# RamSaw/PipelineDP

Hardware: AMD Instinct MI355X
Metric: records/sec DPEngine.aggregate COUNT+SUM at 1/2/4/8 MI355X; % HBM roofline (higher is better)
Workload: dtype f64; 1 GPU; configs[1]: 1e+09 records / 1e+07 privacy ids / 1e+06 Zipf(1.1) partitions per GPU, COUNT+SUM+PRIVACY_ID_COUNT, private partition selection; records_per_gpu=1000000000, privacy_ids_per_gpu=10000000, partitions=1000000, max_partitions_contributed=8, max_contributions_per_partition=2, noise=laplace, selection=truncated_geometric, parallelism=pid-sharded x1, privacy_id_range_supplied=True

## Files before the change

pipelinedp_amd/csrc/dpg_api.hip:

```cpp
#include <dlfcn.h>
#include <hip/hip_runtime.h>
#include <rccl/rccl.h>

#include <algorithm>
#include <cstddef>
#include <chrono>
#include <cmath>
#include <cstdio>
#include <cstdlib>
#include <cstring>
#include <map>
#include <mutex>
#include <string>
#include <thread>
#include <tuple>
#include <vector>

static hipError_t occ_query(int *blocks, const void *kern, int threads, size_t lds) {
    static std::mutex mu;
    static std::map<std::tuple<int, const void *, int, size_t>, int> cache;
    int dev = 0;
    (void)hipGetDevice(&dev);
    std::lock_guard<std::mutex> g(mu);
    const auto key = std::make_tuple(dev, kern, threads, lds);
    const auto it = cache.find(key);
    if (it != cache.end()) {
        *blocks = it->second;
        return hipSuccess;
    }
    const hipError_t e = hipOccupancyMaxActiveBlocksPerMultiprocessor(blocks, kern, threads, lds);
    if (e == hipSuccess) cache[key] = *blocks;
    return e;
}
static hipError_t set_func_attr(const void *kern, hipFuncAttribute attr, int value) {
    if (attr != hipFuncAttributeMaxDynamicSharedMemorySize) return hipFuncSetAttribute(kern, attr, value);
    static std::mutex mu;
    static std::map<std::pair<int, const void *>, int> done;
    int dev = 0;
    (void)hipGetDevice(&dev);
    std::lock_guard<std::mutex> g(mu);
    const auto key = std::make_pair(dev, kern);
    const auto it = done.find(key);
    if (it != done.end() && it->second >= value) return hipSuccess;
    const hipError_t e = hipFuncSetAttribute(kern, attr, value);
    if (e == hipSuccess) done[key] = value;
    return e;
}

#include "dpg_bound.h"
#include "dpg_chunk.h"
#include "dpg_common.h"
#include "dpg_hist.h"
#include "dpg_keydict.h"
#include "dpg_strkey.h"
#include "dpg_owner.h"
#include "dpg_pairx.h"
#include "dpg_partition.h"
#include "dpg_quantile.h"
#include "dpg_records.h"
#include "dpg_rsort.h"
#include "dpg_sample.h"
#include "dpg_select.h"
#include "dpg_shard.h"
#include "dpg_sortb.h"
#include "dpg_sortmw.h"
#include "dpg_team.h"
#include "dpg_utility.h"
#include "dpg_vsum.h"
#include "dpg_wave.h"
#include "dpg_hist_phases.h"

using namespace dpg;

namespace {

constexpr uint32_t kBucketTarget = 256;
constexpr uint32_t kMaxB1 = 11, kMaxB2 = 12, kMaxBR = 11;
constexpr uint32_t kMaxB1W = 12;
constexpr int kIptL1W = 8;
constexpr uint32_t kPinErr = 4096;
constexpr uint32_t kChunkGroup = 32;
constexpr int kRedoLevel2 = -100;
#ifndef DPG_PC_HALF
#define DPG_PC_HALF 0
#endif
#ifndef DPG_IPT_PC
#define DPG_IPT_PC 8
#endif

struct Buf {
    void *p = nullptr;
    size_t bytes = 0;
};

struct Control {
    uint32_t err;
    uint32_t item_cursor;
    uint32_t ntiles[8];
    int64_t n_scalar;
    uint32_t n_chunks;
    uint32_t n_over;
    uint32_t n_over2;
    uint32_t n_mchunks;
    uint32_t heavy_nfb;
    uint32_t pad_;
    uint32_t seg_paths[2];
    unsigned long long over_records;
    unsigned long long over2_records;
    unsigned long long pid_lo, pid_hi;
};

}

struct dpg_ctx {
    int device = 0;
    uint64_t seed = 0;
    int n_cu = 256;
    std::string err;
    std::map<std::string, Buf> bufs;
    std::vector<std::string> stage_names;
    std::vector<hipEvent_t> events;
    int n_events_used = 0;
    hipStream_t last_stream = nullptr;
    uint32_t bucket_target = 0;
    uint32_t bucket_cap = kBCap;
    void *comm = nullptr;
    const uint32_t *last_err = nullptr;
    int rank = 0, nranks = 1;
    char *stage_buf = nullptr;
    size_t stage_cap = 0, stage_head = 0;
    std::map<hipStream_t, hipEvent_t> stage_done;
    uint32_t *pin_tot = nullptr;
    hipEvent_t tot_ev = nullptr;
    uint32_t team_backoff = 0;
    uint32_t team_backoff_next = 64;
};

namespace {

int watchdog_seconds() {
#if defined(DPG_WATCHDOG) || defined(DPG_PHASE_TIMING)
    const char *e = std::getenv("DPG_WATCHDOG_S");
    return e ? std::atoi(e) : 0;
#else
    return 0;
#endif
}

uint32_t *watchdog_buffer(size_t n) {
    static uint32_t *buf = nullptr;
    static size_t cap = 0;
    if (n > cap) {
        if (buf) (void)hipHostFree(buf);
        if (hipHostMalloc((void **)&buf, n * 4, hipHostMallocCoherent) != hipSuccess) return nullptr;
        cap = n;
    }
    std::memset(buf, 0, n * 4);
    return buf;
}

void watchdog_wait(hipStream_t s, const uint32_t *prog, size_t n, const char *what) {
    int secs = watchdog_seconds();
    for (int i = 0; i < secs * 100; ++i) {
        if (hipStreamQuery(s) == hipSuccess) return;
        std::this_thread::sleep_for(std::chrono::milliseconds(10));
    }
    std::fprintf(stderr, "[dpg watchdog] %s did not finish in %d s; phases:", what, secs);
    for (size_t i = 0; i < n; ++i) std::fprintf(stderr, " %u", prog[i]);
    std::fprintf(stderr, "\n");
    std::fflush(stderr);
    std::abort();
// ... 972 lines not shown
    const uint32_t i = blockIdx.x * blockDim.x + threadIdx.x;
    if (i >= 8 * F) return;
    const uint32_t x = i / F, d = i % F;
    rbase[i] = ((int64_t)d * 8 + x) * C;
}

__global__ __launch_bounds__(1024) void k_piece_totals(const uint32_t *cum, const int64_t *rbase,
                                                       uint32_t F, uint32_t *tot, uint32_t *ptot,
                                                       int64_t *ostart, PieceDesc *desc) {
    __shared__ uint32_t sh[16];
    constexpr int DPT = 4;
    const uint32_t d0 = DPT * threadIdx.x;
    uint32_t c[DPT], x = 0;
#pragma unroll
    for (int u = 0; u < DPT; ++u) {
        c[u] = 0;
        uint32_t cp = 0;
        if (d0 + u < F) {
            const uint32_t d = d0 + u;
            const int64_t b0 = rbase[d];
            PieceDesc &pd = desc[d];
            for (int r = 0; r < 8; ++r) {
                const uint32_t y = cum[(size_t)r * F + d];
                pd.ppre[r] = cp;
                pd.dl[r] = (uint32_t)(rbase[(size_t)r * F + d] - b0) - cp;
                pd.cend[r] = cp + y;
                c[u] += y;
                cp += (y + 1u) & ~1u;
            }
            pd.n = cp;
            pd.base0 = b0;
            ptot[d] = cp;
        }
        x += c[u];
    }
    uint32_t total;
    uint32_t e = block_excl_scan_1024(x, sh, total);
#pragma unroll
    for (int u = 0; u < DPT; ++u) {
        if (d0 + u < F) {
            tot[d0 + u] = c[u];
            ostart[d0 + u] = e;
            desc[d0 + u].ostart = e;
        }
        e += c[u];
    }
}

uint32_t piece_capacity(int64_t n, uint32_t F, int64_t sub) {
    double c = 1.25 * (double)n / (8.0 * F) + 4096.0;
    if (const char *e = std::getenv("DPG_DEBUG_PIECE_CAP")) c = std::max(2.0, std::atof(e));
    const double slots = c * 8.0 * F + (double)sub;
    if (slots >= 4294967295.0) return 0;
    return (uint32_t)c & ~1u;
}

template <class R, int IPT, int FMAX, int NT = kScatThreads>
int run_level1_pieces(dpg_ctx *ctx, hipStream_t s, const SrcSoAKey<R, true> &src, int64_t n,
                      uint32_t F, uint32_t bits, uint32_t C, R *out, Control *ctl,
                      PieceTab *pt, uint32_t *host_tot) {
    int st = DPG_OK;
    if (n < 2) return fail(ctx, DPG_ERR_HIP, "internal: piece level needs two records");
    const int64_t sub = (int64_t)NT * IPT;
    const uint32_t nt = (uint32_t)((n + sub - 1) / sub);
    WS(tiles, TileDesc, "pieces.tiles", nt);
    WS(stb, uint32_t, "pieces.stb", 1);
    WS(snt, uint32_t, "pieces.snt", 1);
    WS(rbase, int64_t, "pieces.rbase", (size_t)8 * F);
    WS(cum, uint32_t, "pieces.cum", (size_t)8 * F);
    WS(tot, uint32_t, "pieces.tot", F);
    WS(ptot, uint32_t, "pieces.ptot", F);
    WS(ostart, int64_t, "pieces.ostart", F);
    WS(pdesc, PieceDesc, "pieces.desc", F);
    HIP_TRY(hipMemsetAsync(cum, 0, (size_t)8 * F * 4, s));
    HIP_TRY(hipMemsetAsync(&ctl->ntiles[0], 0, 4, s));
    stage(ctx, s, "partition1:pieces");
    k_region_base<<<(8 * F + 255) / 256, 256, 0, s>>>(rbase, F, C);
    LAUNCH_CHECK();
    k_build_tiles_single<<<(nt + 255) / 256, 256, 0, s>>>(n, sub, 1u, tiles, stb, snt,
                                                         &ctl->ntiles[0], XcdQueues{});
    LAUNCH_CHECK();
    using Src = SrcSoAKey<R, true>;
    constexpr size_t lds = scatter_lds<Src, R, IPT, FMAX, NT>();
    static_assert(lds <= (size_t)160 * 1024 * NT / kScatThreads - 512, "scatter LDS");
    if (F > (uint32_t)FMAX) return fail(ctx, DPG_ERR_HIP, "internal: piece level fan-out too large");
    auto kern = k_scatter<Src, R, IPT, FMAX, false, NT>;
    if (bits <= (uint32_t)agg_bits()) return fail(ctx, DPG_ERR_HIP, "internal: piece level fan-out");
    (void)set_func_attr((const void *)kern, hipFuncAttributeMaxDynamicSharedMemorySize,
                              (int)lds);
    const uint32_t gs = std::min<uint32_t>(nt, (uint32_t)ctx->n_cu * (kScatThreads / NT));
    if (int r = scat_phase_begin(ctx, s)) return r;
    kern<<<gs, NT, lds, s>>>(src, tiles, &ctl->ntiles[0], F, bits, nullptr, rbase, out,
                             XcdQueues{}, nullptr, nullptr, nullptr, 1u, cum, C,
                             (uint32_t)((uint64_t)8 * F * C), &ctl->err);
    LAUNCH_CHECK();
    if (int r = scat_phase_end(ctx, s, "partition1:pieces", gs)) return r;
    k_piece_totals<<<1, 1024, 0, s>>>(cum, rbase, F, tot, ptot, ostart, pdesc);
    LAUNCH_CHECK();
    if (!ctx->tot_ev && hipEventCreateWithFlags(&ctx->tot_ev, hipEventDisableTiming) != hipSuccess)
        return fail(ctx, DPG_ERR_HIP, "hipEventCreate (totals)");
    HIP_TRY(hipMemcpyAsync(host_tot, tot, (size_t)F * 4, hipMemcpyDeviceToHost, s));
    HIP_TRY(hipMemcpyAsync(host_tot + kPinErr, &ctl->err, 4, hipMemcpyDeviceToHost, s));
    HIP_TRY(hipEventRecord(ctx->tot_ev, s));
    *pt = PieceTab{rbase, cum, tot, ptot, ostart, F, pdesc};
    return DPG_OK;
}

template <class R>
int run_team_level2(dpg_ctx *ctx, hipStream_t s, const SrcAoS<R> &src, uint32_t S, uint32_t F2,
                    const int64_t *seg_start, const uint32_t *seg_cnt, R *out, Control *ctl,
                    int64_t **base_out, uint32_t **tot_out, const PieceTab *pt,
                    uint64_t max_bucket) {
    int st = DPG_OK;
    const uint32_t F = kTeamF;
    const size_t words = (size_t)8 * 3 * F + 8 * kTeamArriveStride + 32;
    WS(tw, uint32_t, "team.sync", words);
    WS(base, int64_t, "partition2.base", (size_t)S * F2);
    WS(tot, uint32_t, "partition2.tot", (size_t)S * F2);
    HIP_TRY(hipMemsetAsync(tw, 0, words * 4, s));
    uint32_t *abort_flag = tw + (size_t)8 * 3 * F + 8 * kTeamArriveStride;
    const TeamSync ts{tw, tw + (size_t)8 * 3 * F, abort_flag, &ctl->err};
    if (std::getenv("DPG_DEBUG_TEAM_ABORT")) {
        const uint32_t one = 1;
        UPLOAD(abort_flag, &one, 4);
        k_set_bits<<<1, 1, 0, s>>>(&ctl->err, 8u);
        LAUNCH_CHECK();
    }
    uint32_t sub_cap = (uint32_t)kTeamSub;
    if (const char *e = std::getenv("DPG_DEBUG_TEAM_SUB"))
        sub_cap = std::min<uint32_t>(sub_cap, std::max<uint32_t>(2, (uint32_t)std::atoi(e)) & ~1u);
    const uint32_t T = (uint32_t)ctx->n_cu / 8;
    const bool multi = (max_bucket + 8 + T - 1) / T + 2 > sub_cap;
    const void *k = pt ? (const void *)k_part2_team<R, true> : (const void *)k_part2_team<R, false>;
    (void)set_func_attr(k, hipFuncAttributeMaxDynamicSharedMemorySize, (int)team_lds<R>());
    stage(ctx, s, "partition2:team");
    if (pt)
        k_part2_team<R, true><<<(unsigned)ctx->n_cu, kScatThreads, team_lds<R>(), s>>>(
            src, seg_start, seg_cnt, S, F2, out, base, tot, ts, *pt, sub_cap);
    else
        k_part2_team<R, false><<<(unsigned)ctx->n_cu, kScatThreads, team_lds<R>(), s>>>(
            src, seg_start, seg_cnt, S, F2, out, base, tot, ts, PieceTab{}, sub_cap);
    LAUNCH_CHECK();
    if (multi) {
        stage(ctx, s, "partition2:team_multi");
        HIP_TRY(hipMemsetAsync(tw, 0, ((size_t)8 * 3 * F + 8 * kTeamArriveStride) * 4, s));
        const void *km = pt ? (const void *)k_part2_team<R, true, true>
                            : (const void *)k_part2_team<R, false, true>;
        (void)set_func_attr(km, hipFuncAttributeMaxDynamicSharedMemorySize, (int)team_lds<R>());
        if (pt)
            k_part2_team<R, true, true><<<(unsigned)ctx->n_cu, kScatThreads, team_lds<R>(), s>>>(
                src, seg_start, seg_cnt, S, F2, out, base, tot, ts, *pt, sub_cap);
        else
            k_part2_team<R, false, true><<<(unsigned)ctx->n_cu, kScatThreads, team_lds<R>(), s>>>(
                src, seg_start, seg_cnt, S, F2, out, base, tot, ts, PieceTab{}, sub_cap);
        LAUNCH_CHECK();
    }
    *base_out = base;
    *tot_out = tot;
    return DPG_OK;
}

template <class R>
int pipeline(dpg_ctx *ctx, hipStream_t s, const int64_t *pid, const int64_t *pk,
             const double *value, int64_t n, const dpg_bound_params *p, const dpg_partials *out,
             Control *ctl, const Plan &pl, int64_t pid_min, uint64_t U, uint32_t ib, PaOut *pa) {
    int st = DPG_OK;
    const bool var = (p->metric_mask & (DPG_M_MEAN | DPG_M_VARIANCE)) != 0;
    const Fmt f{ib, pl.pkbits, pl.kbits, pl.b1};
    const HashK H = make_hash(pl.kbits);
    const uint32_t F1 = 1u << pl.b1;
    SrcSoAKey<R> s1{pid, pk, p->public_mask, pl.P, pid_min, U, H, f,
                    low_mask(pl.kbits - pl.b1 + pl.pkbits), pl.kbits - pl.b1, &ctl->err};
    s1.value = value;
    int64_t *bstart = nullptr;
    uint32_t *bcnt = nullptr;
#ifndef DPG_L1_XCD
#define DPG_L1_XCD 0
#endif
#ifndef DPG_L1_SUBS
#define DPG_L1_SUBS 1
#endif
#ifndef DPG_L2_SUBS
#define DPG_L2_SUBS 1
#endif
    auto env_int = [](const char *name, int dflt) {
        const char *e = std::getenv(name);
        return e ? std::atoi(e) : dflt;
    };
    const bool l1_xcd = env_int("DPG_L1_XCD", DPG_L1_XCD) != 0;
    const int l1_subs = env_int("DPG_L1_SUBS", DPG_L1_SUBS);
    const int l2_subs = env_int("DPG_L2_SUBS", DPG_L2_SUBS);
#ifndef DPG_L1_GRP
#define DPG_L1_GRP 1
#endif
#ifndef DPG_L2_GRP
#define DPG_L2_GRP 1
#endif
    const bool l1_grp = env_int("DPG_L1_GRP", DPG_L1_GRP) != 0;
    const bool l2_grp = env_int("DPG_L2_GRP", DPG_L2_GRP) != 0;
    const uint32_t shift2 = pl.pkbits + (pl.kbits - pl.b1) - pl.b2;
    const uint32_t team_T = (uint32_t)ctx->n_cu / 8;
    const bool backoff = ctx->team_backoff > 0;
    if (backoff) {
        --ctx->team_backoff;
        stage(ctx, s, "team_backoff");
    }
    bool team = sizeof(R) == 8 && pl.b2 >= 6 && pl.b2 <= kMaxB1 && ctx->n_cu % 8 == 0 && team_T > 0 && l1_grp &&
                env_int("DPG_TEAM_L2", 1) != 0 && !backoff;
    if constexpr (sizeof(R) != 8) team = false;
    if constexpr (sizeof(R) == 8) if (team) {
        int occ = 0;
        const void *tk = (const void *)k_part2_team<R>;
        (void)set_func_attr(tk, hipFuncAttributeMaxDynamicSharedMemorySize,
                                  (int)team_lds<R>());
        team = occ_query(&occ, tk, kScatThreads,
                                                            team_lds<R>()) == hipSuccess &&
               occ >= 1;
    }
    if (team && !ctx->pin_tot &&
        hipHostMalloc((void **)&ctx->pin_tot, (size_t)4 * (kPinErr + 64), hipHostMallocDefault) != hipSuccess) {
        ctx->pin_tot = nullptr;
        team = false;
    }
    constexpr int kIptPc = DPG_IPT_PC;
    const bool pc_half = F1 <= 2048 && env_int("DPG_PC_HALF", DPG_PC_HALF) != 0;
    const int64_t subPc = (int64_t)(pc_half ? kScatThreads / 2 : kScatThreads) *
                          (F1 > 2048 ? kIptL1W : kIptPc);
    uint32_t pcap = 0;
    bool pieces = false;
    if constexpr (sizeof(R) == 8) {
        if (team && env_int("DPG_L1_PIECES", 1) != 0 && n >= ((int64_t)1 << 22) &&
            pl.b1 > (uint32_t)agg_bits()) {
            pcap = piece_capacity(n, F1, subPc);
            pieces = pcap > 0;
        }
    }
    WS(recA, R, "recA", pieces ? std::max<int64_t>(n, (int64_t)8 * F1 * pcap + subPc) : n);
    WS(recB, R, "recB", n);
    int64_t *bstart1 = nullptr;
    uint32_t *bcnt1 = nullptr;
    auto level1_std = [&](bool with_tot) -> int {
        if constexpr (sizeof(R) == 8) {
            if (F1 > 2048)
                return run_level<SrcSoAKey<R>, R, kIptL1W, 4096>(
                    ctx, s, s1, 1u, nullptr, nullptr, &ctl->n_scalar, n, F1, pl.b1, recA,
                    "partition1", &bstart1, &bcnt1, &ctl->ntiles[0], nullptr, l1_xcd, l1_subs,
                    l1_grp, with_tot ? ctx->pin_tot : nullptr);
        }
        return run_level<SrcSoAKey<R>, R, Ipt<R>::L1, 2048>(
            ctx, s, s1, 1u, nullptr, nullptr, &ctl->n_scalar, n, F1, pl.b1, recA, "partition1",
            &bstart1, &bcnt1, &ctl->ntiles[0], nullptr, l1_xcd, l1_subs, l1_grp,
            with_tot ? ctx->pin_tot : nullptr);
    };
    PieceTab ptab{};
    uint64_t max_bucket = 0;
    int r = DPG_OK;
    if constexpr (sizeof(R) == 8) {
        if (pieces) {
            SrcSoAKey<R, true> sp{pid, pk, p->public_mask, pl.P, pid_min, U, H, f,
                                  low_mask(pl.kbits - pl.b1 + pl.pkbits), pl.kbits - pl.b1,
                                  &ctl->err};
            r = F1 > 2048 ? run_level1_pieces<R, kIptL1W, 4096>(ctx, s, sp, n, F1, pl.b1, pcap, recA,
                                                               ctl, &ptab, ctx->pin_tot)
                : pc_half ? run_level1_pieces<R, kIptPc, 2048, kScatThreads / 2>(
                                ctx, s, sp, n, F1, pl.b1, pcap, recA, ctl, &ptab, ctx->pin_tot)
                          : run_level1_pieces<R, kIptPc, 2048>(ctx, s, sp, n, F1, pl.b1, pcap, recA,
                                                               ctl, &ptab, ctx->pin_tot);
            if (r) return r;
            HIP_TRY(hipEventSynchronize(ctx->tot_ev));
            for (uint32_t d = 0; d < F1; ++d) max_bucket = std::max<uint64_t>(max_bucket, ctx->pin_tot[d]);
            const bool over = (ctx->pin_tot[kPinErr] & 16u) != 0;
            if (over) {
                std::fprintf(stderr, "[dpg] histogram-free level 1: a region overflowed; redone "
                                     "with the histogram path\n");
                HIP_TRY(hipMemsetAsync(&ctl->err, 0, 4, s));
                pieces = false;
                max_bucket = 0;
            }
        }
    }
    if (!pieces) {
        r = level1_std(team);
        if (r) return r;
        if (team) {
            HIP_TRY(hipEventSynchronize(ctx->tot_ev));
            for (uint32_t d = 0; d < F1; ++d) max_bucket = std::max<uint64_t>(max_bucket, ctx->pin_tot[d]);
        }
    }
    bstart = bstart1;
    bcnt = bcnt1;
    const R *cur = recA;
    uint32_t B = F1;
    auto level2_grouped = [&]() -> int {
        const uint32_t F2 = 1u << pl.b2;
        SrcAoS<R> s2{recA, f, shift2, F2 - 1};
#ifndef DPG_L2_XCD
#define DPG_L2_XCD 1
#endif
        int r = pl.b2 > 11
                ? run_level<SrcAoS<R>, R, Ipt<R>::LW, 4096>(ctx, s, s2, F1, bstart1, bcnt1, nullptr, n,
                                                             F2, pl.b2, recB, "partition2", &bstart,
                                                             &bcnt, &ctl->ntiles[1], nullptr,
                                                             DPG_L2_XCD != 0, l2_subs, l2_grp)
                : run_level<SrcAoS<R>, R, Ipt<R>::LN, 2048>(ctx, s, s2, F1, bstart1, bcnt1, nullptr, n,
                                                             F2, pl.b2, recB, "partition2", &bstart,
                                                             &bcnt, &ctl->ntiles[1], nullptr,
                                                             DPG_L2_XCD != 0, l2_subs, l2_grp);
        return r;
    };
    if (pl.b2 > 0) {
        const uint32_t F2 = 1u << pl.b2;
        if constexpr (sizeof(R) == 8) {
            if (team) {
                SrcAoS<R> s2{recA, f, shift2, F2 - 1};
                r = run_team_level2<R>(ctx, s, s2, F1, F2, bstart1, bcnt1, recB, ctl, &bstart, &bcnt,
                                       pieces ? &ptab : nullptr, max_bucket);
            }
        }
        if (!team) {
            r = level2_grouped();
        }
        if (r) return r;
        cur = recB;
        B = F1 * F2;
    }
    BoundParams bp = to_bound(p, stream_seed(ctx->seed, p->nonce));
    bp.fmt = f;
    bp.hash = H;
    bp.pid_min = pid_min;
    bp.value = value;
    bp.err = &ctl->err;
    const bool key32 = pl.pkbits <= 21;
    auto bound = [&]() -> int {
        if (pa)
            return key32 ? bound_and_reduce<R, uint32_t, ItemPA>(ctx, s, pl, cur, bstart, bcnt, B, bp,
                                                                 n, out, ctl, pa)
                         : bound_and_reduce<R, uint64_t, ItemPA>(ctx, s, pl, cur, bstart, bcnt, B, bp,
                                                                 n, out, ctl, pa);
        if constexpr (sizeof(R) == 16) {
            return fail(ctx, DPG_ERR_HIP, "internal: R16 outside the pre-aggregate");
        } else {
            if (var && !(p->metric_mask & DPG_M_SUM) && p->sum_mode != DPG_SUM_CLIP_PARTITION)
                return key32 ? bound_and_reduce<R, uint32_t, ItemV>(ctx, s, pl, cur, bstart, bcnt, B,
                                                                    bp, n, out, ctl, nullptr)
                             : bound_and_reduce<R, uint64_t, ItemV>(ctx, s, pl, cur, bstart, bcnt, B,
                                                                    bp, n, out, ctl, nullptr);
            if (var)
                return key32 ? bound_and_reduce<R, uint32_t, Item32>(ctx, s, pl, cur, bstart, bcnt, B,
                                                                     bp, n, out, ctl, nullptr)
                             : bound_and_reduce<R, uint64_t, Item32>(ctx, s, pl, cur, bstart, bcnt, B,
// ... 1908 lines not shown
```

pipelinedp_amd/csrc/dpg_partition.h:

```cpp
#pragma once

#include "dpg_common.h"

#include <type_traits>

namespace dpg {

#ifndef DPG_HIST_U
#define DPG_HIST_U 8
#endif
#ifndef DPG_SCAT_WB
#define DPG_SCAT_WB 2
#endif
constexpr int kPartThreads = 1024;
constexpr int kScatThreads = 1024;

__host__ __device__ constexpr size_t a16(size_t x) { return (x + 15) & ~(size_t)15; }

typedef int64_t i64x2 __attribute__((ext_vector_type(2)));
typedef uint64_t u64x2 __attribute__((ext_vector_type(2)));
typedef uint64_t u64x2a8 __attribute__((ext_vector_type(2), aligned(8)));
typedef uint32_t u32x2 __attribute__((ext_vector_type(2)));
typedef uint32_t u32x4 __attribute__((ext_vector_type(4)));

// ... 750 lines not shown
__device__ __forceinline__ uint32_t scatter_scan_update(uint32_t *cnt, uint32_t *dstart,
                                                        uint32_t *cur, uint32_t F,
                                                        uint32_t *sh16, uint32_t *goff = nullptr,
                                                        uint32_t cap = 0, uint32_t dump = 0,
                                                        uint32_t *err = nullptr,
                                                        const uint32_t *lb = nullptr) {
    constexpr int NW = T / 64;
    const uint32_t d0 = DPT * threadIdx.x;
    uint32_t c[DPT], x = 0;
#pragma unroll
    for (int u = 0; u < DPT; ++u) {
        c[u] = d0 + u < F ? cnt[d0 + u] : 0u;
        x += c[u];
    }
    constexpr bool kPair = DPT == 2 && DPG_SCAT_RSV_PAIR;
    uint32_t o[DPT];
    if constexpr (kPair && DPG_SCAT_RSV_PAIR_EARLY) {
        if (goff && d0 < F) {
            const unsigned long long old = atomicAdd(
                reinterpret_cast<unsigned long long *>(&goff[d0]),
                (unsigned long long)c[0] | ((unsigned long long)c[1] << 32));
            o[0] = (uint32_t)old;
            o[1] = (uint32_t)(old >> 32);
        }
    }
    const int lane = threadIdx.x & 63, w = threadIdx.x >> 6;
    uint32_t wt;
    uint32_t e = wave_excl_scan(x, wt);
    if (lane == 63) sh16[w] = wt;
    __syncthreads();
    uint32_t total = 0;
#pragma unroll
    for (int k = 0; k < NW; ++k) {
        const uint32_t y = sh16[k];
        if (k < w) e += y;
        total += y;
    }
    if constexpr (kPair && !DPG_SCAT_RSV_PAIR_EARLY) {
        if (goff && d0 < F) {
            const unsigned long long old = atomicAdd(
                reinterpret_cast<unsigned long long *>(&goff[d0]),
                (unsigned long long)c[0] | ((unsigned long long)c[1] << 32));
            o[0] = (uint32_t)old;
            o[1] = (uint32_t)(old >> 32);
        }
    }
#pragma unroll
    for (int u = 0; u < DPT; ++u) {
        if (d0 + u < F) {
            dstart[d0 + u] = e;
            if constexpr (kCap) {
                if (c[u]) {
                    const uint32_t ou = kPair ? o[u] : atomicAdd(&goff[d0 + u], c[u]);
                    if (ou + c[u] <= cap) {
                        cur[d0 + u] = (lb ? lb[d0 + u] : cur[d0 + u]) + ou + c[u];
                    } else {
                        cur[d0 + u] = dump + e + c[u];
                        atomicOr(err, 16u);
                    }
                }
            } else if (goff) {
                if (c[u]) cur[d0 + u] += (kPair ? o[u] : atomicAdd(&goff[d0 + u], c[u])) + c[u];
            } else {
                cur[d0 + u] += c[u];
            }
            cnt[d0 + u] = 0;
        }
        e += c[u];
    }
    if (threadIdx.x == 0) dstart[F] = total;
    __syncthreads();
    return total;
}

template <int DPT>
struct PcRsv {
    uint32_t c[DPT];
    uint32_t e0;
    unsigned long long old[DPT / 2];
};
struct NoBetween {
    __device__ __forceinline__ void operator()() const {}
};
template <int NT, int DPT, class Between = NoBetween>
__device__ __forceinline__ uint32_t scatter_scan_pc(uint32_t *cnt, uint32_t *dstart, uint32_t F,
                                                    uint32_t *sh16, uint32_t *goff, PcRsv<DPT> &r,
                                                    Between between = Between{}) {
    const uint32_t d0 = DPT * threadIdx.x;
    uint32_t x = 0;
#pragma unroll
    for (int u = 0; u < DPT; ++u) {
        r.c[u] = d0 + u < F ? cnt[d0 + u] : 0u;
        x += r.c[u];
    }
#pragma unroll
    for (int q = 0; q < DPT / 2; ++q)
        r.old[q] = atomicAdd(reinterpret_cast<unsigned long long *>(&goff[(d0 + 2 * q) % F]),
                             (unsigned long long)r.c[2 * q] | ((unsigned long long)r.c[2 * q + 1] << 32));
    between();
    const int lane = threadIdx.x & 63, w = threadIdx.x >> 6;
    uint32_t wt;
    uint32_t e = wave_excl_scan(x, wt);
    if (lane == 63) sh16[w] = wt;
    __syncthreads();
    uint32_t total = 0;
#pragma unroll
    for (int k = 0; k < NT / 64; ++k) {
        const uint32_t y = sh16[k];
        if (k < w) e += y;
        total += y;
    }
    r.e0 = e;
#pragma unroll
    for (int u = 0; u < DPT; ++u) {
        if (d0 + u < F) {
            dstart[d0 + u] = e;
            cnt[d0 + u] = 0;
        }
        e += r.c[u];
    }
    if (threadIdx.x == 0) dstart[F] = total;
    __syncthreads();
    return total;
}
template <int DPT>
__device__ __forceinline__ void scatter_rsv_finish(const PcRsv<DPT> &r, uint32_t *cur,
                                                   const uint32_t *lb, uint32_t F, uint32_t cap,
                                                   uint32_t dump, uint32_t *err) {
    const uint32_t d0 = DPT * threadIdx.x;
    uint32_t o[DPT];
#pragma unroll
    for (int q = 0; q < DPT / 2; ++q) {
        o[2 * q] = (uint32_t)r.old[q];
        o[2 * q + 1] = (uint32_t)(r.old[q] >> 32);
    }
    uint32_t e = r.e0;
    bool over = false;
#pragma unroll
    for (int u = 0; u < DPT; ++u) {
        const bool fits = o[u] + r.c[u] <= cap;
        const uint32_t v = fits ? (lb[d0 + u < F ? d0 + u : 0u] + o[u] + r.c[u]) : dump + e + r.c[u];
        if (d0 + u < F && r.c[u]) {
            cur[d0 + u] = v;
            over = over || !fits;
        }
        e += r.c[u];
    }
    if (over) atomicOr(err, 16u);
}

__global__ __launch_bounds__(1024) void k_digit_base(const int64_t *seg_start, uint32_t F,
                                                     const uint32_t *tot, int64_t *base) {
    __shared__ uint32_t sh[16];
    const uint32_t s = blockIdx.x;
    const uint32_t d0 = 4 * threadIdx.x;
    uint32_t c[4], x = 0;
#pragma unroll
    for (int u = 0; u < 4; ++u) {
        c[u] = d0 + u < F ? tot[(size_t)s * F + d0 + u] : 0u;
        x += c[u];
    }
    uint32_t total;
    uint32_t e = block_excl_scan_1024(x, sh, total);
    const int64_t st = seg_start ? seg_start[s] : 0;
#pragma unroll
    for (int u = 0; u < 4; ++u) {
        if (d0 + u < F) base[(size_t)s * F + d0 + u] = st + e;
        e += c[u];
    }
}

__device__ __forceinline__ uint32_t wave_agg_rank(uint32_t *cnt, uint32_t d, bool ok,
                                                  uint32_t bits) {
    uint64_t peers = __ballot(ok);
    for (uint32_t b = 0; b < bits; ++b) {
        uint64_t bal = __ballot((d >> b) & 1u);
        peers &= ((d >> b) & 1u) ? bal : ~bal;
    }
    const int lane = __lane_id();
    const int leader = peers ? __ffsll((long long)peers) - 1 : lane;
    const uint32_t below = __popcll(peers & ((1ull << lane) - 1ull));
    uint32_t basev = 0;
    if (ok && lane == leader) basev = atomicAdd(&cnt[d], (uint32_t)__popcll(peers));
    basev = __shfl(basev, leader, 64);
    return basev + below;
}

template <class T, int kW = (sizeof(T) % 16 == 0 ? 16 : sizeof(T) % 8 == 0 ? 8 : 4)>
struct Words {
    static constexpr int N = sizeof(T) / 16;
    uint4 w[N];
};
template <class T>
struct Words<T, 8> {
    static constexpr int N = sizeof(T) / 8;
    uint2 w[N];
};
template <class T>
struct Words<T, 4> {
    static constexpr int N = sizeof(T) / 4;
    uint32_t w[N];
};
template <class T>
__device__ __forceinline__ Words<T> to_words(const T &r) {
    Words<T> x;
    __builtin_memcpy(&x, &r, sizeof(T));
    return x;
}
template <class T>
__device__ __forceinline__ T from_words(const Words<T> &x) {
    T r;
    __builtin_memcpy(&r, &x, sizeof(T));
    return r;
}

template <class Src, class Rec, int IPT, int FMAX, int NT = kScatThreads>
constexpr size_t scatter_lds_core() {
    return (size_t)sizeof(Rec) * (NT * IPT + 1) +
           (Src::kDigitFromRec ? 0 : a16((size_t)2 * (NT * IPT + 1))) +
           (size_t)FMAX * 12 + 80;
}
#ifndef DPG_SCAT_LBASE
#define DPG_SCAT_LBASE 1
#endif
#ifndef DPG_PC_NORESET
#define DPG_PC_NORESET 1
#endif
#ifndef DPG_PC_LATE_RSV
#define DPG_PC_LATE_RSV 1
#endif
#ifndef DPG_L1_PF
#define DPG_L1_PF 2
#endif
template <class Src, class Rec, int IPT, int FMAX, int NT = kScatThreads>
constexpr bool scatter_lbase() {
    return scatter_lds_core<Src, Rec, IPT, FMAX, NT>() + (size_t)FMAX * 4 <= 160 * 1024;
}
template <class Src, class Rec, int IPT, int FMAX, int NT = kScatThreads>
constexpr size_t scatter_lds() {
    return scatter_lds_core<Src, Rec, IPT, FMAX, NT>() +
           (scatter_lbase<Src, Rec, IPT, FMAX, NT>() ? (size_t)FMAX * 4 : 0);
}

#ifdef DPG_PHASE_TIMING
__device__ unsigned long long g_scat_cyc[8];
#define DPG_SCAT_MARK(k)                                         \
    do {                                                         \
        if (threadIdx.x == 0) {                                  \
            const uint64_t now_ = __builtin_amdgcn_s_memtime();  \
            scyc[k] += now_ - slast;                             \
            slast = now_;                                        \
        }                                                        \
    } while (0)
#else
#define DPG_SCAT_MARK(k) \
    do {                 \
    } while (0)
#endif

template <class Src, class Rec, int IPT, int FMAX, bool kAgg, int NT = kScatThreads>
__global__ __launch_bounds__(NT, 4) void k_scatter(Src src_in, const TileDesc *tiles,
                                                          const uint32_t *ntiles, uint32_t F,
                                                          uint32_t bits, const uint32_t *off,
                                                          const int64_t *base, Rec *out,
                                                          XcdQueues xq = XcdQueues{},
                                                          const uint32_t *cbase = nullptr,
                                                          const uint32_t *seg_tile_base = nullptr,
                                                          const uint32_t *seg_ntiles = nullptr,
                                                          uint32_t C = 1, uint32_t *goff = nullptr,
                                                          uint32_t pcap = 0, uint32_t pdump = 0,
                                                          uint32_t *perr = nullptr) {
    constexpr int SUB = NT * IPT;
    constexpr bool kPc = HasPieces<Src>::value;
    constexpr bool kSD = !Src::kDigitFromRec;
    constexpr bool kP = HasFetchPairs<Src>::value && IPT % 2 == 0;
    constexpr bool kEarly = kPc && kP && DPG_L1_PF != 0;
    constexpr int kPF = kEarly ? DPG_L1_PF : 0;
    using W = Words<Rec>;
    extern __shared__ __attribute__((aligned(16))) char smem[];
    W *stage = reinterpret_cast<W *>(smem);
    uint16_t *sdig = reinterpret_cast<uint16_t *>(smem + sizeof(Rec) * (SUB + 1));
    const size_t o = sizeof(Rec) * (SUB + 1) + (kSD ? a16((size_t)2 * (SUB + 1)) : 0);
    uint32_t *cnt = reinterpret_cast<uint32_t *>(smem + o);
    uint32_t *dstart = cnt + FMAX;
    uint32_t *cur = dstart + FMAX + 1;
    uint32_t *sh16 = cur + FMAX;
    constexpr bool kLB = DPG_SCAT_LBASE && scatter_lbase<Src, Rec, IPT, FMAX, NT>();
    uint32_t *lbase = reinterpret_cast<uint32_t *>(smem + scatter_lds_core<Src, Rec, IPT, FMAX, NT>());
    uint32_t lseg = 0xFFFFFFFFu;

    const uint32_t nt = __builtin_amdgcn_readfirstlane(*ntiles);
    const int tid = threadIdx.x;
    auto elem = [tid](int j) -> uint32_t {
        return kP ? (uint32_t)((j >> 1) * 2 * NT + 2 * tid + (j & 1))
                  : (uint32_t)(j * NT + tid);
    };
    __shared__ uint32_t sh_next;
    const uint32_t xq_id = blockIdx.x & 7u;
    const uint32_t xq_len = xq.q ? __builtin_amdgcn_readfirstlane(xq.n[xq_id]) : 0u;
    constexpr uint32_t kNone = 0xFFFFFFFFu;
    Src src = src_in;
    typename Src::Raw raw[IPT];
    constexpr bool kSeg = HasRegions<Src>::value;
    bool seg_fast = true;
    auto load_sub = [&](int64_t b0, uint32_t lim) {
        if constexpr (kEarly) {
#pragma unroll
            for (int m = 0; m < IPT / 2; ++m) {
                const int32_t o = m * 2 * NT + 2 * tid;
                src.fetch2(b0 + min(o, (int32_t)lim - 2), raw[2 * m], raw[2 * m + 1]);
            }
            return;
        } else if constexpr (kP) {
            if (lim >= 2) {
#pragma unroll
                for (int m = 0; m < IPT / 2; ++m) {
                    const uint32_t o = m * 2 * NT + 2 * tid;
                    const uint32_t a = min(o, lim - 2);
                    typename Src::Raw x0, x1;
                    src.fetch2(b0 + a, x0, x1);
                    raw[2 * m] = a == o ? x0 : x1;
                    raw[2 * m + 1] = x1;
                }
                return;
            }
        }
        if constexpr (kSeg) {
            seg_fast = src.fetch_sub(b0, lim, b0 + SUB, elem, raw);
            return;
        }
#pragma unroll
        for (int j = 0; j < IPT; ++j) raw[j] = src.fetch(b0 + min(elem(j), lim - 1));
    };
    auto decode_raw = [&](int j, uint32_t lim, int64_t i, Rec &r, uint32_t &d) -> bool {
        if constexpr (kEarly) {
            if ((j & 1) == 0)
                return src.decode((int32_t)elem(j) > (int32_t)lim - 2 ? raw[j + 1] : raw[j], i, r, d);
        }
        return src.decode(raw[j], i, r, d);
    };
    uint32_t it = blockIdx.x;
    uint32_t t = kNone;
    if (xq.q) {
        if (tid == 0) sh_next = atomicAdd(&xq.next[xq_id], 1u);
// ... 18 lines not shown
            cnt[d] = 0;
        }
        __syncthreads();
    }
    for (;;) {
    uint32_t nq = 0;
    const uint32_t *cb = nullptr;
    uint32_t *gof = goff ? goff + (size_t)(kPc ? (blockIdx.x & 7u) : td.pad) * F : nullptr;
    if constexpr (!kPcLB) {
    if (xq.q && tid == 0) nq = atomicAdd(&xq.next[xq_id], 1u);
    __syncthreads();
    if (cbase) {
        const uint32_t nta = seg_ntiles[td.seg], per = (nta + C - 1) / C;
        cb = cbase + ((size_t)td.seg * C + (t - seg_tile_base[td.seg]) / per) * F;
    }
    const uint32_t bsel = kPc ? (blockIdx.x & 7u) : td.seg;
    if (kLB && goff) {
        if (bsel != lseg) {
            for (uint32_t d = tid; d < F; d += NT) lbase[d] = (uint32_t)base[(size_t)bsel * F + d];
            lseg = bsel;
        }
        for (uint32_t d = tid; d < F; d += NT) {
            cur[d] = lbase[d];
            cnt[d] = 0;
        }
    } else {
        for (uint32_t d = tid; d < F; d += NT) {
            cur[d] = (uint32_t)(base[(size_t)bsel * F + d] +
                                (goff ? 0u : off[(size_t)t * F + d] + (cb ? cb[d] : 0u)));
            cnt[d] = 0;
        }
    }
    __syncthreads();
    }
    uint32_t tn = kNone;
    TileDesc tdn = td;
    DPG_SCAT_MARK(4);
    for (int64_t sb = td.begin; sb < td.end; sb += SUB) {
        const uint32_t lim = (uint32_t)min<int64_t>(SUB, td.end - sb);
        Rec rec[IPT];
        uint32_t dr[IPT];
        if constexpr (kSeg) {
            if (!seg_fast) {
#pragma unroll
                for (int j = 0; j < IPT; ++j) raw[j] = src.fetch(sb + min(elem(j), lim - 1));
            }
            if (src.paths && tid == 0) atomicAdd(&src.paths[seg_fast ? 0 : 1], 1u);
        }
        if constexpr (!kAgg) {
            uint32_t dg[IPT];
            bool okv[IPT];
#pragma unroll
            for (int j = 0; j < IPT; ++j) {
                const uint32_t o = elem(j);
                uint32_t d = 0;
                if constexpr (kEarly)
                    okv[j] = o < lim && decode_raw(j, lim, sb + o, rec[j], d);
                else
                    okv[j] = o < lim && src.decode(raw[j], sb + o, rec[j], d);
                dg[j] = okv[j] ? d : 0u;
            }
            uint32_t rk[IPT];
#pragma unroll
            for (int j = 0; j < IPT; ++j) rk[j] = atomicAdd(&cnt[dg[j]], okv[j] ? 1u : 0u);
#pragma unroll
            for (int j = 0; j < IPT; ++j) dr[j] = okv[j] ? (dg[j] | (rk[j] << 12)) : ~0u;
        } else {
#pragma unroll
            for (int j = 0; j < IPT; ++j) {
                const uint32_t o = elem(j);
                uint32_t d = 0;
                bool ok;
                if constexpr (kEarly)
                    ok = o < lim && decode_raw(j, lim, sb + o, rec[j], d);
                else
                    ok = o < lim && src.decode(raw[j], sb + o, rec[j], d);
                const uint32_t rk = wave_agg_rank(cnt, ok ? d : 0u, ok, bits);
                dr[j] = ok ? (d | (rk << 12)) : ~0u;
            }
        }
        if (xq.q && tid == 0 && sb == td.begin) sh_next = nq;
        __syncthreads();
        DPG_SCAT_MARK(0);
        constexpr int kDPT = FMAX / NT;
        constexpr bool kLate = kPcLB && (kDPT == 2 || kDPT == 4) && FMAX == kDPT * NT && DPG_PC_LATE_RSV;
        PcRsv<(kDPT >= 2 ? kDPT : 2)> rsv;
        uint32_t total;
        if constexpr (!kEarly) {
        if constexpr (kLate)
            total = scatter_scan_pc<NT, kDPT>(cnt, dstart, F, sh16, gof, rsv);
        else
            total = scatter_scan_update<NT, FMAX / NT, kPc>(
                cnt, dstart, cur, F, sh16, gof, pcap, pdump, perr, kPcLB ? lbase : nullptr);
        DPG_SCAT_MARK(1);
        {
            uint32_t ds[IPT];
#pragma unroll
            for (int j = 0; j < IPT; ++j) ds[j] = dstart[dr[j] != ~0u ? (dr[j] & 0xFFFu) : 0u];
#pragma unroll
            for (int j = 0; j < IPT; ++j) {
                const uint32_t pos = dr[j] != ~0u ? ds[j] + (dr[j] >> 12) : (uint32_t)SUB;
                stage[pos] = to_words(rec[j]);
                if constexpr (kSD) sdig[pos] = (uint16_t)(dr[j] & 0xFFFu);
            }
        }
        if constexpr (kLate) scatter_rsv_finish(rsv, cur, lbase, F, pcap, pdump, perr);
        __syncthreads();
        DPG_SCAT_MARK(2);
        const int64_t nb = sb + SUB;
        const uint32_t nlim = (uint32_t)max<int64_t>(0, min<int64_t>(SUB, td.end - nb));
        {
            int64_t lb = nb;
            uint32_t ll = nlim;
            if constexpr (HasTilePrefetch<Src>::value && kPc) {
                if (nlim == 0 && it + gridDim.x < nt) {
                    tn = it + gridDim.x;
                    tdn.begin = (int64_t)tn * SUB;
                    tdn.end = min(tdn.begin + SUB, n_end);
                    lb = tdn.begin;
                    ll = (uint32_t)min<int64_t>(SUB, tdn.end - tdn.begin);
                }
            } else if constexpr (HasTilePrefetch<Src>::value) {
                if (nlim == 0 && xq.q) {
                    const uint32_t w = __builtin_amdgcn_readfirstlane(sh_next);
                    if (w < xq_len) {
                        tn = __builtin_amdgcn_readfirstlane(xq.q[(size_t)xq_id * xq.stride + w]);
                        tdn = uniform_tile(tiles, tn);
                        lb = tdn.begin;
                        ll = (uint32_t)min<int64_t>(SUB, tdn.end - tdn.begin);
                    }
                }
            }
            if (ll > 0) load_sub(lb, ll);
        }
        } else {
        auto prefetch = [&]() {
            const int64_t nb = sb + SUB;
            const uint32_t nlim = (uint32_t)max<int64_t>(0, min<int64_t>(SUB, td.end - nb));
            int64_t lb = nb;
            uint32_t ll = nlim;
            if (nlim == 0) {
                lb = sb;
                ll = lim;
                if (it + gridDim.x < nt) {
                    tn = it + gridDim.x;
                    tdn.begin = (int64_t)tn * SUB;
                    tdn.end = min(tdn.begin + SUB, n_end);
                    lb = tdn.begin;
                    ll = (uint32_t)min<int64_t>(SUB, tdn.end - tdn.begin);
                }
            }
            load_sub(lb, ll);
        };
        if constexpr (kLate && kPF == 3) {
            total = scatter_scan_pc<NT, kDPT>(cnt, dstart, F, sh16, gof, rsv, prefetch);
        } else {
            if constexpr (kLate)
                total = scatter_scan_pc<NT, kDPT>(cnt, dstart, F, sh16, gof, rsv);
            else
                total = scatter_scan_update<NT, FMAX / NT, kPc>(
                    cnt, dstart, cur, F, sh16, gof, pcap, pdump, perr, kPcLB ? lbase : nullptr);
            prefetch();
        }
        DPG_SCAT_MARK(1);
        {
            uint32_t ds[IPT];
#pragma unroll
            for (int j = 0; j < IPT; ++j) ds[j] = dstart[dr[j] != ~0u ? (dr[j] & 0xFFFu) : 0u];
#pragma unroll
            for (int j = 0; j < IPT; ++j) {
                const uint32_t pos = dr[j] != ~0u ? ds[j] + (dr[j] >> 12) : (uint32_t)SUB;
                stage[pos] = to_words(rec[j]);
                if constexpr (kSD) sdig[pos] = (uint16_t)(dr[j] & 0xFFFu);
            }
        }
        if constexpr (kLate) scatter_rsv_finish(rsv, cur, lbase, F, pcap, pdump, perr);
        __syncthreads();
        DPG_SCAT_MARK(2);
        }
        constexpr int WB = IPT < DPG_SCAT_WB ? IPT : DPG_SCAT_WB;
        constexpr int kWbIter = (IPT + WB - 1) / WB;
        auto write_batch = [&](uint32_t k0) {
            W x[WB];
            static_assert(!kSeg || sizeof(W) / W::N >= 8, "items are read as 8- or 16-byte words");
            using NV = std::conditional_t<sizeof(W) / W::N == 16, u32x4, u32x2>;
            NV xv[WB][W::N];
            uint32_t dd[WB], kc[WB];
#pragma unroll
            for (int u = 0; u < WB; ++u) {
                kc[u] = min(k0 + u * NT + tid, total - 1);
                if constexpr (kSeg) {
#pragma unroll
                    for (int q = 0; q < W::N; ++q)
                        xv[u][q] = reinterpret_cast<const NV *>(&stage[kc[u]])[q];
                } else {
                    x[u] = stage[kc[u]];
                }
                if constexpr (kSD) dd[u] = sdig[kc[u]];
            }
            if constexpr (kSeg) {
#pragma unroll
                for (int u = 0; u < WB; ++u) {
                    dd[u] = src.digit_word0(xv[u][0].x);
                }
            } else if constexpr (!kSD) {
#pragma unroll
                for (int u = 0; u < WB; ++u) dd[u] = src.digit(from_words<Rec>(x[u]));
            }
            uint32_t c1[WB], c2[WB];
#pragma unroll
            for (int u = 0; u < WB; ++u) {
                c1[u] = cur[dd[u]];
                c2[u] = dstart[dd[u] + 1];
            }
#if DPG_EXP_SCAT_NOSTORE
#pragma unroll
            for (int u = 0; u < WB; ++u) {
                uint32_t w0;
                __builtin_memcpy(&w0, &x[u], 4);
                if (w0 == 0x12345u && c1[u] == 0x777u)
                    *reinterpret_cast<W *>(&out[c1[u] - c2[u] + kc[u]]) = x[u];
            }
#else
#pragma unroll
            for (int u = 0; u < WB; ++u) {
                W *dst = reinterpret_cast<W *>(&out[c1[u] - c2[u] + kc[u]]);
                if constexpr (kSeg) {
#pragma unroll
                    for (int q = 0; q < W::N; ++q) reinterpret_cast<NV *>(dst)[q] = xv[u][q];
                } else {
                    *dst = x[u];
                }
            }
#endif
        };
        if constexpr (kPc || kSeg) {
#pragma unroll
            for (int b = 0; b < kWbIter; ++b) {
                if ((uint32_t)b * WB * NT >= total) break;
                write_batch((uint32_t)b * WB * NT);
            }
        } else {
            for (uint32_t k0 = 0; k0 < total; k0 += WB * NT) write_batch(k0);
        }
        DPG_SCAT_MARK(3);
#ifdef DPG_PHASE_TIMING
        if (tid == 0) ++scyc[5];
#endif
    }
    if (!HasTilePrefetch<Src>::value && xq.q) {
        const uint32_t w = __builtin_amdgcn_readfirstlane(sh_next);
        if (w >= xq_len) break;
        tn = __builtin_amdgcn_readfirstlane(xq.q[(size_t)xq_id * xq.stride + w]);
        tdn = uniform_tile(tiles, tn);
        load_sub(tdn.begin, (uint32_t)min<int64_t>(SUB, tdn.end - tdn.begin));
    } else if (kPc && HasTilePrefetch<Src>::value) {
        it += gridDim.x;
    } else if (!xq.q) {
        it += gridDim.x;
// ... 17 lines not shown
```

Baseline: 56.93 billion records/s.

## Parameterize piece-level scatter workgroup size and derive occupancy from LDS

Adds a DPG_PC_NT knob (default 1024) for the level-1 piece scatter, decoupling its thread count from the half-mode path. Workgroups per CU and launch bounds are now computed from LDS usage instead of a fixed value. Scatter_scan_pc and rsv_finish gain a path for digit-per-thread counts that don't evenly cover FMAX. The staging write loop is batched to limit register pressure. The aim is a better occupancy and register tradeoff in the piece scatter, at the cost of new edge cases when F is not a power of two.

```diff
diff --git a/pipelinedp_amd/csrc/dpg_api.hip b/pipelinedp_amd/csrc/dpg_api.hip
--- a/pipelinedp_amd/csrc/dpg_api.hip
+++ b/pipelinedp_amd/csrc/dpg_api.hip
@@ -87,6 +87,10 @@
 #ifndef DPG_IPT_PC
 #define DPG_IPT_PC 8
 #endif
+#ifndef DPG_PC_NT
+#define DPG_PC_NT 1024
+#endif
+static_assert(DPG_PC_NT % 64 == 0 && DPG_PC_NT <= 1024 && DPG_IPT_PC % 2 == 0, "piece level shape");
 
 struct Buf {
     void *p = nullptr;
@@ -1225,13 +1229,16 @@
     LAUNCH_CHECK();
     using Src = SrcSoAKey<R, true>;
     constexpr size_t lds = scatter_lds<Src, R, IPT, FMAX, NT>();
-    static_assert(lds <= (size_t)160 * 1024 * NT / kScatThreads - 512, "scatter LDS");
+    constexpr int wg_cu = scatter_wg_per_cu<Src, R, IPT, FMAX, NT>();
+    static_assert(lds <= (size_t)160 * 1024 / wg_cu - 512, "scatter LDS");
+    static_assert(sub < (1 << 20), "sub-tile ranks are kept in 20 bits (k_scatter's dr[])");
     if (F > (uint32_t)FMAX) return fail(ctx, DPG_ERR_HIP, "internal: piece level fan-out too large");
+    if (F < 4 || (F & (F - 1))) return fail(ctx, DPG_ERR_HIP, "internal: piece level fan-out");
     auto kern = k_scatter<Src, R, IPT, FMAX, false, NT>;
     if (bits <= (uint32_t)agg_bits()) return fail(ctx, DPG_ERR_HIP, "internal: piece level fan-out");
     (void)set_func_attr((const void *)kern, hipFuncAttributeMaxDynamicSharedMemorySize,
                               (int)lds);
-    const uint32_t gs = std::min<uint32_t>(nt, (uint32_t)ctx->n_cu * (kScatThreads / NT));
+    const uint32_t gs = std::min<uint32_t>(nt, (uint32_t)ctx->n_cu * wg_cu);
     if (int r = scat_phase_begin(ctx, s)) return r;
     kern<<<gs, NT, lds, s>>>(src, tiles, &ctl->ntiles[0], F, bits, nullptr, rbase, out,
                              XcdQueues{}, nullptr, nullptr, nullptr, 1u, cum, C,
@@ -1365,15 +1372,17 @@
         ctx->pin_tot = nullptr;
         team = false;
     }
-    constexpr int kIptPc = DPG_IPT_PC;
+    constexpr int kIptPc = DPG_IPT_PC, kNtPc = DPG_PC_NT;
+    constexpr int kIptHalf = 8, kNtHalf = kScatThreads / 2;
     const bool pc_half = F1 <= 2048 && env_int("DPG_PC_HALF", DPG_PC_HALF) != 0;
-    const int64_t subPc = (int64_t)(pc_half ? kScatThreads / 2 : kScatThreads) *
-                          (F1 > 2048 ? kIptL1W : kIptPc);
+    const int64_t subPc = F1 > 2048 ? (int64_t)kScatThreads * kIptL1W
+                          : pc_half ? (int64_t)kNtHalf * kIptHalf
+                                    : (int64_t)kNtPc * kIptPc;
     uint32_t pcap = 0;
     bool pieces = false;
     if constexpr (sizeof(R) == 8) {
         if (team && env_int("DPG_L1_PIECES", 1) != 0 && n >= ((int64_t)1 << 22) &&
-            pl.b1 > (uint32_t)agg_bits()) {
+            pl.b1 > (uint32_t)agg_bits() && pl.b1 >= 2) {
             pcap = piece_capacity(n, F1, subPc);
             pieces = pcap > 0;
         }
@@ -1405,10 +1414,10 @@
                                   &ctl->err};
             r = F1 > 2048 ? run_level1_pieces<R, kIptL1W, 4096>(ctx, s, sp, n, F1, pl.b1, pcap, recA,
                                                                ctl, &ptab, ctx->pin_tot)
-                : pc_half ? run_level1_pieces<R, kIptPc, 2048, kScatThreads / 2>(
+                : pc_half ? run_level1_pieces<R, kIptHalf, 2048, kNtHalf>(
                                 ctx, s, sp, n, F1, pl.b1, pcap, recA, ctl, &ptab, ctx->pin_tot)
-                          : run_level1_pieces<R, kIptPc, 2048>(ctx, s, sp, n, F1, pl.b1, pcap, recA,
-                                                               ctl, &ptab, ctx->pin_tot);
+                          : run_level1_pieces<R, kIptPc, 2048, kNtPc>(
+                                ctx, s, sp, n, F1, pl.b1, pcap, recA, ctl, &ptab, ctx->pin_tot);
             if (r) return r;
             HIP_TRY(hipEventSynchronize(ctx->tot_ev));
             for (uint32_t d = 0; d < F1; ++d) max_bucket = std::max<uint64_t>(max_bucket, ctx->pin_tot[d]);
diff --git a/pipelinedp_amd/csrc/dpg_partition.h b/pipelinedp_amd/csrc/dpg_partition.h
--- a/pipelinedp_amd/csrc/dpg_partition.h
+++ b/pipelinedp_amd/csrc/dpg_partition.h
@@ -856,20 +856,34 @@
 struct NoBetween {
     __device__ __forceinline__ void operator()() const {}
 };
-template <int NT, int DPT, class Between = NoBetween>
+template <int NT, int DPT, bool kOne = false, class Between = NoBetween>
 __device__ __forceinline__ uint32_t scatter_scan_pc(uint32_t *cnt, uint32_t *dstart, uint32_t F,
                                                     uint32_t *sh16, uint32_t *goff, PcRsv<DPT> &r,
                                                     Between between = Between{}) {
     const uint32_t d0 = DPT * threadIdx.x;
     uint32_t x = 0;
+    if constexpr (kOne) {
+#pragma unroll
+        for (int u = 0; u < DPT; ++u) r.c[u] = 0u;
+        if (d0 < F) {
+#pragma unroll
+            for (int u = 0; u < DPT; ++u) r.c[u] = cnt[d0 + u];
+        }
+#pragma unroll
+        for (int u = 0; u < DPT; ++u) x += r.c[u];
+    } else {
 #pragma unroll
     for (int u = 0; u < DPT; ++u) {
         r.c[u] = d0 + u < F ? cnt[d0 + u] : 0u;
         x += r.c[u];
     }
+    }
+    if constexpr (kOne) __builtin_assume(F <= (uint32_t)(DPT * NT));
+    const uint32_t g0 = kOne ? d0 & (F - 1) : 0u;
 #pragma unroll
     for (int q = 0; q < DPT / 2; ++q)
-        r.old[q] = atomicAdd(reinterpret_cast<unsigned long long *>(&goff[(d0 + 2 * q) % F]),
+        r.old[q] = atomicAdd(reinterpret_cast<unsigned long long *>(
+                                 &goff[kOne ? g0 + 2 * q : (d0 + 2 * q) % F]),
                              (unsigned long long)r.c[2 * q] | ((unsigned long long)r.c[2 * q + 1] << 32));
     between();
     const int lane = threadIdx.x & 63, w = threadIdx.x >> 6;
@@ -885,6 +899,16 @@
         total += y;
     }
     r.e0 = e;
+    if constexpr (kOne) {
+        if (d0 < F) {
+#pragma unroll
+            for (int u = 0; u < DPT; ++u) {
+                dstart[d0 + u] = e;
+                cnt[d0 + u] = 0;
+                e += r.c[u];
+            }
+        }
+    } else {
 #pragma unroll
     for (int u = 0; u < DPT; ++u) {
         if (d0 + u < F) {
@@ -893,11 +917,12 @@
         }
         e += r.c[u];
     }
+    }
     if (threadIdx.x == 0) dstart[F] = total;
     __syncthreads();
     return total;
 }
-template <int DPT>
+template <int DPT, bool kOne = false>
 __device__ __forceinline__ void scatter_rsv_finish(const PcRsv<DPT> &r, uint32_t *cur,
                                                    const uint32_t *lb, uint32_t F, uint32_t cap,
                                                    uint32_t dump, uint32_t *err) {
@@ -910,6 +935,21 @@
     }
     uint32_t e = r.e0;
     bool over = false;
+    if constexpr (kOne) {
+        const uint32_t db = d0 < F ? d0 : 0u;
+#pragma unroll
+        for (int u = 0; u < DPT; ++u) {
+            const bool fits = o[u] + r.c[u] <= cap;
+            const uint32_t v = fits ? lb[db + u] + o[u] + r.c[u] : dump + e + r.c[u];
+            if (d0 < F && r.c[u]) {
+                cur[d0 + u] = v;
+                over = over || !fits;
+            }
+            e += r.c[u];
+        }
+        if (over) atomicOr(err, 16u);
+        return;
+    }
 #pragma unroll
     for (int u = 0; u < DPT; ++u) {
         const bool fits = o[u] + r.c[u] <= cap;
@@ -1006,6 +1046,9 @@
 #ifndef DPG_L1_PF
 #define DPG_L1_PF 2
 #endif
+#ifndef DPG_PC_STAGE_B
+#define DPG_PC_STAGE_B 8
+#endif
 template <class Src, class Rec, int IPT, int FMAX, int NT = kScatThreads>
 constexpr bool scatter_lbase() {
     return scatter_lds_core<Src, Rec, IPT, FMAX, NT>() + (size_t)FMAX * 4 <= 160 * 1024;
@@ -1014,6 +1057,18 @@
 constexpr size_t scatter_lds() {
     return scatter_lds_core<Src, Rec, IPT, FMAX, NT>() +
            (scatter_lbase<Src, Rec, IPT, FMAX, NT>() ? (size_t)FMAX * 4 : 0);
+}
+
+template <class Src, class Rec, int IPT, int FMAX, int NT = kScatThreads>
+constexpr int scatter_wg_per_cu() {
+    const size_t by_lds = (size_t)160 * 1024 / (scatter_lds<Src, Rec, IPT, FMAX, NT>() + 512);
+    const size_t by_thr = kScatThreads / NT;
+    const size_t w = by_lds < by_thr ? by_lds : by_thr;
+    return w < 1 ? 1 : (int)w;
+}
+template <class Src, class Rec, int IPT, int FMAX, int NT = kScatThreads>
+constexpr int scatter_waves_per_simd() {
+    return (scatter_wg_per_cu<Src, Rec, IPT, FMAX, NT>() * (NT / 64) + 3) / 4;
 }
 
 #ifdef DPG_PHASE_TIMING
@@ -1033,7 +1088,8 @@
 #endif
 
 template <class Src, class Rec, int IPT, int FMAX, bool kAgg, int NT = kScatThreads>
-__global__ __launch_bounds__(NT, 4) void k_scatter(Src src_in, const TileDesc *tiles,
+__global__ __launch_bounds__(NT, (scatter_waves_per_simd<Src, Rec, IPT, FMAX, NT>()))
+void k_scatter(Src src_in, const TileDesc *tiles,
                                                           const uint32_t *ntiles, uint32_t F,
                                                           uint32_t bits, const uint32_t *off,
                                                           const int64_t *base, Rec *out,
@@ -1218,13 +1274,14 @@
         if (xq.q && tid == 0 && sb == td.begin) sh_next = nq;
         __syncthreads();
         DPG_SCAT_MARK(0);
-        constexpr int kDPT = FMAX / NT;
-        constexpr bool kLate = kPcLB && (kDPT == 2 || kDPT == 4) && FMAX == kDPT * NT && DPG_PC_LATE_RSV;
-        PcRsv<(kDPT >= 2 ? kDPT : 2)> rsv;
+        constexpr int kDPT = ((FMAX + NT - 1) / NT + 1) & ~1;
+        constexpr bool kLate = kPcLB && (kDPT == 2 || kDPT == 4) && DPG_PC_LATE_RSV;
+        constexpr bool kOne = kDPT * NT != FMAX;
+        PcRsv<kDPT> rsv;
         uint32_t total;
         if constexpr (!kEarly) {
         if constexpr (kLate)
-            total = scatter_scan_pc<NT, kDPT>(cnt, dstart, F, sh16, gof, rsv);
+            total = scatter_scan_pc<NT, kDPT, kOne>(cnt, dstart, F, sh16, gof, rsv);
         else
             total = scatter_scan_update<NT, FMAX / NT, kPc>(
                 cnt, dstart, cur, F, sh16, gof, pcap, pdump, perr, kPcLB ? lbase : nullptr);
@@ -1240,7 +1297,7 @@
                 if constexpr (kSD) sdig[pos] = (uint16_t)(dr[j] & 0xFFFu);
             }
         }
-        if constexpr (kLate) scatter_rsv_finish(rsv, cur, lbase, F, pcap, pdump, perr);
+        if constexpr (kLate) scatter_rsv_finish<kDPT, kOne>(rsv, cur, lbase, F, pcap, pdump, perr);
         __syncthreads();
         DPG_SCAT_MARK(2);
         const int64_t nb = sb + SUB;
@@ -1289,10 +1346,10 @@
             load_sub(lb, ll);
         };
         if constexpr (kLate && kPF == 3) {
-            total = scatter_scan_pc<NT, kDPT>(cnt, dstart, F, sh16, gof, rsv, prefetch);
+            total = scatter_scan_pc<NT, kDPT, kOne>(cnt, dstart, F, sh16, gof, rsv, prefetch);
         } else {
             if constexpr (kLate)
-                total = scatter_scan_pc<NT, kDPT>(cnt, dstart, F, sh16, gof, rsv);
+                total = scatter_scan_pc<NT, kDPT, kOne>(cnt, dstart, F, sh16, gof, rsv);
             else
                 total = scatter_scan_update<NT, FMAX / NT, kPc>(
                     cnt, dstart, cur, F, sh16, gof, pcap, pdump, perr, kPcLB ? lbase : nullptr);
@@ -1300,17 +1357,25 @@
         }
         DPG_SCAT_MARK(1);
         {
-            uint32_t ds[IPT];
-#pragma unroll
-            for (int j = 0; j < IPT; ++j) ds[j] = dstart[dr[j] != ~0u ? (dr[j] & 0xFFFu) : 0u];
-#pragma unroll
-            for (int j = 0; j < IPT; ++j) {
-                const uint32_t pos = dr[j] != ~0u ? ds[j] + (dr[j] >> 12) : (uint32_t)SUB;
-                stage[pos] = to_words(rec[j]);
-                if constexpr (kSD) sdig[pos] = (uint16_t)(dr[j] & 0xFFFu);
-            }
-        }
-        if constexpr (kLate) scatter_rsv_finish(rsv, cur, lbase, F, pcap, pdump, perr);
+            constexpr int kSB = DPG_PC_STAGE_B > 0 && DPG_PC_STAGE_B < IPT ? DPG_PC_STAGE_B : IPT;
+#pragma unroll
+            for (int j0 = 0; j0 < IPT; j0 += kSB) {
+                uint32_t ds[kSB];
+#pragma unroll
+                for (int j = 0; j < kSB; ++j)
+                    if (j0 + j < IPT) ds[j] = dstart[dr[j0 + j] != ~0u ? (dr[j0 + j] & 0xFFFu) : 0u];
+#pragma unroll
+                for (int j = 0; j < kSB; ++j) {
+                    if (j0 + j < IPT) {
+                        const uint32_t pos =
+                            dr[j0 + j] != ~0u ? ds[j] + (dr[j0 + j] >> 12) : (uint32_t)SUB;
+                        stage[pos] = to_words(rec[j0 + j]);
+                        if constexpr (kSD) sdig[pos] = (uint16_t)(dr[j0 + j] & 0xFFFu);
+                    }
+                }
+            }
+        }
+        if constexpr (kLate) scatter_rsv_finish<kDPT, kOne>(rsv, cur, lbase, F, pcap, pdump, perr);
         __syncthreads();
         DPG_SCAT_MARK(2);
         }
```

Result: no change. 56.79 billion records/s (median of 2 runs) (-0.3%).
